# hvak/visual-underwater-slam

Measured on AMD Instinct MI355X. Metric: ORB detect+match frames/sec, higher is better.
Workload: dtype u8

## Files before the change

visual-underwater-slam_amd/csrc/orient.hip:

```cpp
#include "frontend_common.h"
#include <type_traits>
#define VUS_TABLE_QUAL __device__ constexpr
#include "../../include/vus_orb_tables.h"
#include "../../include/vus_tiled.h"

namespace {

#ifndef VUS_OR_WPE
#define VUS_OR_WPE 4
#endif
#ifndef VUS_OR_WPE_TILED
#define VUS_OR_WPE_TILED 7
#endif
constexpr int OR_R = 15;
constexpr int OR_ROWS = 2 * OR_R + 1;
constexpr int OR_DW = 10;
constexpr int BR_R = VUS_RBRIEF_REACH;
constexpr int BR_ROWS = 2 * BR_R + 1;
constexpr int BR_DW = 10;
constexpr int BR_DW_TILED = 16;
constexpr int OR_PC = 3;
constexpr int OR_NP = OR_ROWS * OR_PC;
constexpr int OR_KP_PER_WAVE = 8;

typedef uint32_t PatchVec __attribute__((ext_vector_type(2), aligned(1)));

template <int RADIUS, int DW, bool EXACT>
struct PatchRegs {
  static_assert(DW % 2 == 0, "row width must be a multiple of the vector width");
  static constexpr int ROWS = 2 * RADIUS + 1;
  static constexpr int HW = DW / 2;
  static constexpr int N = ROWS * HW;
  static constexpr int ITERS = (N + 63) / 64;
  PatchVec v[ITERS];
  uint32_t off[ITERS];

  __device__ __forceinline__ void init(int pitch, int lane) {
#pragma unroll
    for (int u = 0; u < ITERS; ++u) {
      const int t = min(lane + 64 * u, N - 1);
      off[u] = (uint32_t)((t / HW) * pitch + 8 * (t % HW));
    }
  }
  __device__ __forceinline__ void load(const uint8_t* __restrict__ src, int H, int W, int pitch, int y, int x,
                                       int lane) {
    const int xa = EXACT ? x - RADIUS : (x - RADIUS) & ~3;
    const bool inside = y - RADIUS >= 0 && y + RADIUS < H && xa >= 0 && xa + 4 * DW <= W;
    if (inside) {
      const uint8_t* base = src + (size_t)(y - RADIUS) * pitch + xa;
#pragma unroll
      for (int u = 0; u < ITERS; ++u) v[u] = *reinterpret_cast<const PatchVec*>(base + (size_t)off[u]);
    } else {
#pragma unroll
      for (int u = 0; u < ITERS; ++u) {
        const int t = min(lane + 64 * u, N - 1);
        const int r = t / HW, c = t - r * HW;
        const uint8_t* rp = src + (size_t)clampi(y - RADIUS + r, 0, H - 1) * pitch;
        const int gx = xa + 8 * c;
#pragma unroll
        for (int k = 0; k < 2; ++k)
          v[u][k] = (uint32_t)rp[clampi(gx + 4 * k, 0, W - 1)] | ((uint32_t)rp[clampi(gx + 4 * k + 1, 0, W - 1)] << 8) |
                    ((uint32_t)rp[clampi(gx + 4 * k + 2, 0, W - 1)] << 16) |
                    ((uint32_t)rp[clampi(gx + 4 * k + 3, 0, W - 1)] << 24);
      }
    }
  }
  __device__ __forceinline__ void store(uint32_t* __restrict__ dst, int lane) const {
#pragma unroll
    for (int u = 0; u < ITERS; ++u)
      if (lane + 64 * u < N) *reinterpret_cast<uint2*>(dst + 2 * (lane + 64 * u)) = make_uint2(v[u][0], v[u][1]);
  }
};

__device__ __forceinline__ uint4 tiled_piece_clamped(const uint8_t* __restrict__ src, int H, int W, int gy, int gx) {
  gy = clampi(gy, 0, H - 1);
  uint32_t w[4];
#pragma unroll
  for (int j = 0; j < 4; ++j) {
    w[j] = 0;
#pragma unroll
    for (int b = 0; b < 4; ++b) w[j] |= (uint32_t)src[vus_tiled_offset(gy, clampi(gx + 4 * j + b, 0, W - 1), W)] << (8 * b);
  }
  return make_uint4(w[0], w[1], w[2], w[3]);
}

struct PieceRC {
  int r, c;
};
constexpr int BR_PC = 3;
__host__ __device__ constexpr PieceRC disc_piece(int q) {
  const int c = (q >= OR_ROWS ? 1 : 0) + (q >= 2 * OR_ROWS ? 1 : 0);
  return {q - OR_ROWS * c, c};
}
constexpr int BR_SLOTS = 12 * ((BR_ROWS + 3) / 4);
__host__ __device__ constexpr PieceRC brief_piece(int t) {
  const int g = (t * 171) >> 11, w = t - 12 * g;
  return {4 * g + (w & 3), w >> 2};
}
template <int ROWS, int PC, int SLOTS, PieceRC (*PIECE)(int)>
constexpr bool dealing_is_a_permutation() {
  bool seen[ROWS * PC] = {};
  int n = 0;
  for (int s = 0; s < SLOTS; ++s) {
    const PieceRC p = PIECE(s);
    if (p.r < 0 || p.c < 0 || p.c >= PC) return false;
    if (p.r >= ROWS) continue;
    if (seen[p.r * PC + p.c]) return false;
    seen[p.r * PC + p.c] = true;
    ++n;
  }
  return n == ROWS * PC;
}
static_assert(dealing_is_a_permutation<OR_ROWS, OR_PC, OR_NP, disc_piece>(), "centroid patch: 31 x 3 pieces, one slot each");
static_assert(dealing_is_a_permutation<BR_ROWS, BR_PC, BR_SLOTS, brief_piece>(), "descriptor patch: 37 x 3 pieces, one slot each");
static_assert(BR_SLOTS <= 128, "descriptor patch: two wave-loads");

struct TiledDiscPair {
  static constexpr int ITERS = (2 * OR_NP + 63) / 64;
  static constexpr int SPLIT = OR_NP - 64;
  static_assert(ITERS == 3 && SPLIT > 0 && SPLIT < 64, "wave-load 1 is the only mixed one");
  static constexpr int PK_OFF_BITS = 10, PK_IDX_SHIFT = 10, PK_IDX_BITS = 10, PK_ROW_SHIFT = 20, PK_ROW_BITS = 6;
  static_assert(16 * (OR_ROWS - 1) + 128 * (OR_PC - 1) < (1 << PK_OFF_BITS) && PK_OFF_BITS <= PK_IDX_SHIFT, "pk: the offset field");
  static_assert(OR_NP - 1 < (1 << PK_IDX_BITS) && PK_IDX_SHIFT + PK_IDX_BITS <= PK_ROW_SHIFT, "pk: the weight index field");
  static_assert(OR_ROWS - 1 + 7 < (1 << PK_ROW_BITS) && PK_ROW_SHIFT + PK_ROW_BITS <= 32, "pk: the row field, nothing above it");
  uint4 v[ITERS];
  uint32_t pk[ITERS];

  static __device__ __forceinline__ int slot_of(int p) { return p >= OR_NP ? p - OR_NP : p; }
  __device__ __forceinline__ void init(int , int lane) {
#pragma unroll
    for (int u = 0; u < ITERS; ++u) {
      const PieceRC pc = disc_piece(slot_of(min(lane + 64 * u, 2 * OR_NP - 1)));
      const uint32_t r = (uint32_t)pc.r, c = (uint32_t)pc.c;
      pk[u] = r << PK_ROW_SHIFT | (OR_PC * r + c) << PK_IDX_SHIFT | (16u * r + 128u * c);
    }
  }
  __device__ __forceinline__ int row(int u) const { return (int)(pk[u] >> PK_ROW_SHIFT); }
  __device__ __forceinline__ int weight_index(int u) const { return (int)((pk[u] >> PK_IDX_SHIFT) & ((1u << PK_IDX_BITS) - 1u)); }
  static __device__ __forceinline__ bool inside(int H, int W, int y, int x) {
    const int xa = (x - OR_R) & ~15;
    return y - OR_R >= 0 && y + OR_R < H && xa >= 0 && xa + 16 * OR_PC <= W;
  }
  __device__ __forceinline__ void load(const uint8_t* __restrict__ src, int H, int W, int ya, int xa, int yb, int xb, bool b_live,
                                       int lane) {
    const bool second = lane >= SPLIT;
    const bool idle2 = lane >= 2 * OR_NP - 128;
    if (inside(H, W, ya, xa) && (!b_live || inside(H, W, yb, xb))) {
      const int y0a = ya - OR_R, y0b = yb - OR_R;
      const uint32_t koa = vus_tiled_offset(y0a & ~7, (xa - OR_R) & ~15, W) + 16u * (uint32_t)(y0a & 7);
      const uint32_t kob = b_live ? vus_tiled_offset(y0b & ~7, (xb - OR_R) & ~15, W) + 16u * (uint32_t)(y0b & 7) : koa;
      const uint32_t ysa = (uint32_t)(y0a & 7) << PK_ROW_SHIFT, ysb = (uint32_t)(y0b & 7) << PK_ROW_SHIFT, ystep = 8u * (uint32_t)W - 128u;
      constexpr int BLK = PK_ROW_SHIFT + 3;
      constexpr uint32_t OFF = (1u << PK_OFF_BITS) - 1u;
      v[0] = *reinterpret_cast<const uint4*>(src + koa + (size_t)(((pk[0] + ysa) >> BLK) * ystep + (pk[0] & OFF)));
      v[1] = make_uint4(0u, 0u, 0u, 0u);
      v[2] = make_uint4(0u, 0u, 0u, 0u);
      if (!second || b_live)
        v[1] = *reinterpret_cast<const uint4*>(
            src + (size_t)((second ? kob : koa) + ((pk[1] + (second ? ysb : ysa)) >> BLK) * ystep + (pk[1] & OFF)));
      if (b_live && !idle2)
        v[2] = *reinterpret_cast<const uint4*>(src + kob + (size_t)(((pk[2] + ysb) >> BLK) * ystep + (pk[2] & OFF)));
    } else {
#pragma unroll
      for (int u = 0; u < ITERS; ++u) {
        const int p = lane + 64 * u;
        const bool sec = p >= OR_NP;
        const PieceRC pc = disc_piece(slot_of(min(p, 2 * OR_NP - 1)));
        const int y = sec ? yb : ya, x = sec ? xb : xa;
        v[u] = make_uint4(0u, 0u, 0u, 0u);
        if (p < 2 * OR_NP && (!sec || b_live)) v[u] = tiled_piece_clamped(src, H, W, y - OR_R + pc.r, ((x - OR_R) & ~15) + 16 * pc.c);
      }
    }
  }
};

struct TiledBriefRegs {
  static constexpr int ROWS = BR_ROWS;
  uint4 v[2];
  uint32_t col;

  static __device__ __forceinline__ bool wide(int x) { return ((x - BR_R) & 15) > 11; }
  static __device__ __forceinline__ PieceRC loaded_piece(int lane, int u) {
    const PieceRC p = brief_piece(min(lane + 64 * u, BR_SLOTS - 1));
    return {min(p.r, ROWS - 1), p.c};
  }
  __device__ __forceinline__ void init(int , int ) { col = 0; }
  __device__ __forceinline__ void load(const uint8_t* __restrict__ src, int H, int W, int , int y, int x, int lane) {
    const int xa = (x - BR_R) & ~15, y0 = y - BR_R, rc = min(lane, ROWS - 1);
    const bool inside = y0 >= 0 && y + BR_R < H && xa >= 0 && xa + (wide(x) ? 64 : 48) <= W;
    if (inside) {
      const uint8_t* base = src + vus_tiled_offset(y0 & ~7, xa, W) + 16 * (y0 & 7);
      const uint32_t ys = (uint32_t)(y0 & 7), ystep = 8u * (uint32_t)W - 128u;
#pragma unroll
      for (int u = 0; u < 2; ++u) {
        const PieceRC p = loaded_piece(lane, u);
        const uint32_t off = (((uint32_t)p.r + ys) >> 3) * ystep + 16u * (uint32_t)p.r + 128u * (uint32_t)p.c;
        v[u] = *reinterpret_cast<const uint4*>(base + (size_t)off);
      }
      if (wide(x))
        col = *reinterpret_cast<const uint32_t*>(base + (size_t)((((uint32_t)rc + ys) >> 3) * ystep + 16u * (uint32_t)rc + 384u));
    } else {
#pragma unroll
      for (int u = 0; u < 2; ++u) {
        const PieceRC p = loaded_piece(lane, u);
        v[u] = tiled_piece_clamped(src, H, W, y0 + p.r, xa + 16 * p.c);
      }
      if (wide(x)) {
        const int gy = clampi(y0 + rc, 0, H - 1);
        uint32_t w = 0;
#pragma unroll
        for (int b = 0; b < 4; ++b) w |= (uint32_t)src[vus_tiled_offset(gy, clampi(xa + 48 + b, 0, W - 1), W)] << (8 * b);
        col = w;
      }
    }
  }
  __device__ __forceinline__ void store(uint32_t* __restrict__ dst, int lane, int x) const {
    uint4* d = reinterpret_cast<uint4*>(dst);
#pragma unroll
    for (int u = 0; u < 2; ++u) {
      const int t = lane + 64 * u;
      const PieceRC p = brief_piece(min(t, BR_SLOTS - 1));
      if (t < BR_SLOTS && p.r < ROWS) d[(BR_DW_TILED / 4) * p.r + p.c] = v[u];
    }
    if (wide(x) && lane < ROWS) dst[16 * lane + 12] = col;
  }
};

__device__ __forceinline__ int fold32(int x, int y) {
  auto r = __builtin_amdgcn_permlane32_swap((uint32_t)x, (uint32_t)y, false, false);
  return (int)(r[0] + r[1]);
}
__device__ __forceinline__ int fold16(int x, int y) {
  auto r = __builtin_amdgcn_permlane16_swap((uint32_t)x, (uint32_t)y, false, false);
  return (int)(r[0] + r[1]);
}
template <int CTRL>
__device__ __forceinline__ int dpp_i32(int v) { return __builtin_amdgcn_update_dpp(0, v, CTRL, 0xf, 0xf, true); }
constexpr int DPP_ROW_ROR8 = 0x128, DPP_HALF_MIRROR = 0x141, DPP_QUAD_XOR1 = 0xB1, DPP_QUAD_XOR2 = 0x4E;
__device__ __forceinline__ int fold8(int x, int y, bool upper8) {
  const int keep = upper8 ? y : x, give = upper8 ? x : y;
  return keep + dpp_i32<DPP_ROW_ROR8>(give);
}
__device__ __forceinline__ int allsum8(int v) {
  v += dpp_i32<DPP_HALF_MIRROR>(v);
  v += dpp_i32<DPP_QUAD_XOR1>(v);
  v += dpp_i32<DPP_QUAD_XOR2>(v);
  return v;
}
template <int CTRL>
__device__ __forceinline__ long long dpp_max_i64(long long key) {
  const int lo = dpp_i32<CTRL>((int)(uint32_t)key), hi = dpp_i32<CTRL>((int)(key >> 32));
  const long long ok = (long long)(((unsigned long long)(uint32_t)hi << 32) | (uint32_t)lo);
  return ok > key ? ok : key;
}
__device__ __forceinline__ long long allmax8_i64(long long key) {
  key = dpp_max_i64<DPP_HALF_MIRROR>(key);
  key = dpp_max_i64<DPP_QUAD_XOR1>(key);
  key = dpp_max_i64<DPP_QUAD_XOR2>(key);
  return key;
}

__device__ __forceinline__ uint32_t writelane_u32(uint32_t reg, uint32_t value, int lane_sel) {
  asm("s_mov_b32 m0, %2\n\tv_writelane_b32 %0, %1, m0" : "+v"(reg) : "s"(value), "s"(lane_sel));
  return reg;
}

__device__ __forceinline__ void load_bin_directions(const int (&cos_table)[VUS_N_ANGLE_BINS], const int (&sin_table)[VUS_N_ANGLE_BINS],
                                                    int lane, int (&bin_cos)[4], int (&bin_sin)[4]) {
#pragma unroll
  for (int q = 0; q < 4; ++q) {
    const int bq = min(4 * (lane & 7) + q, VUS_N_ANGLE_BINS - 1);
    bin_cos[q] = cos_table[bq];
    bin_sin[q] = sin_table[bq];
  }
}

struct RotOffTable {
  uint32_t v[VUS_N_ANGLE_BINS * 64 * 4];
};
constexpr RotOffTable make_rot_off_table(int row_bytes) {
  RotOffTable r{};
  for (int e = 0; e < VUS_N_ANGLE_BINS * 256; ++e) {
    const int bin = e / 256, test = e - 256 * bin, w = test >> 6, lane = test & 63;
    const int oa = VUS_RBRIEF_ROT[4 * e + 1] * row_bytes + VUS_RBRIEF_ROT[4 * e];
    const int ob = VUS_RBRIEF_ROT[4 * e + 3] * row_bytes + VUS_RBRIEF_ROT[4 * e + 2];
    r.v[(bin * 64 + lane) * 4 + w] = ((uint32_t)oa & 0xFFFFu) | ((uint32_t)ob << 16);
  }
  return r;
}
__device__ __attribute__((aligned(128))) const RotOffTable g_rot_off_table = make_rot_off_table(4 * BR_DW);
__device__ __attribute__((aligned(128))) const RotOffTable g_rot_off_table_tiled = make_rot_off_table(4 * BR_DW_TILED);

constexpr int OR_NV = OR_ROWS * (OR_DW / 2);
constexpr int OR_WT = 192;

template <int ALIGN>
struct DiscWeightTable {
  uint32_t v[ALIGN * OR_WT * 4];
};
struct DiscDwordWeight {
  uint32_t moment, count;
};
constexpr DiscDwordWeight disc_dword_weight(int dy, int dx0) {
  constexpr int umax[16] = {15, 15, 15, 15, 14, 14, 14, 13, 13, 12, 11, 10, 9, 8, 6, 3};
  DiscDwordWeight w{0u, 0u};
  if (dy < -OR_R || dy > OR_R) return w;
  const int um = umax[dy < 0 ? -dy : dy];
  for (int b = 0; b < 4; ++b) {
    const int dx = dx0 + b;
    if (dx >= -um && dx <= um) {
      w.moment |= (uint32_t)(dx + OR_R) << (8 * b);
      w.count |= 1u << (8 * b);
    }
  }
  return w;
}
template <int ALIGN>
constexpr DiscWeightTable<ALIGN> make_disc_weight_table() {
  DiscWeightTable<ALIGN> r{};
  for (int e = 0; e < ALIGN * OR_WT; ++e) {
    const int sh = e / OR_WT, t = e - sh * OR_WT;
    if (t >= OR_NV) continue;
    const int row = t / (OR_DW / 2), c = t - row * (OR_DW / 2);
    for (int d = 0; d < 2; ++d) {
      const DiscDwordWeight w = disc_dword_weight(row - OR_R, 4 * (2 * c + d) - sh - OR_R);
      r.v[4 * e + d] = w.moment;
      r.v[4 * e + 2 + d] = w.count;
    }
  }
  return r;
}
__device__ __attribute__((aligned(128))) const DiscWeightTable<4> g_disc_weight_table = make_disc_weight_table<4>();

constexpr int OR_WTD = 3 + 4 * (3 * 64 - OR_NP) + 4;
struct DiscWeightDwTable {
  uint32_t v[4 * OR_WTD * 2];
};
constexpr DiscWeightDwTable make_disc_weight_dw_table() {
  DiscWeightDwTable r{};
  for (int e = 0; e < 4 * OR_WTD; ++e) {
    const int a = e / OR_WTD, d = e - a * OR_WTD - 3;
    if (d < 0 || d >= OR_ROWS * 4 * OR_PC) continue;
    const int row = d / (4 * OR_PC), col = d - row * (4 * OR_PC);
    const DiscDwordWeight w = disc_dword_weight(row - OR_R, 4 * col - a - OR_R);
    r.v[2 * e] = w.moment;
    r.v[2 * e + 1] = w.count;
  }
  return r;
}
__device__ __attribute__((aligned(128))) const DiscWeightDwTable g_disc_weight_dw_table = make_disc_weight_dw_table();
constexpr bool disc_weight_dw_table_matches() {
  constexpr DiscWeightDwTable dw = make_disc_weight_dw_table();
  for (int sh = 0; sh < 16; ++sh)
    for (int q = 0; q < 3 * 64 - OR_NP; ++q)
      for (int d = 0; d < 4; ++d) {
        const int e = (sh & 3) * OR_WTD + 4 * q + d + 3 - (sh >> 2);
        const int r = q / OR_PC, c = q - r * OR_PC;
        const DiscDwordWeight w = disc_dword_weight(r - OR_R, 16 * c + 4 * d - sh - OR_R);
        if (dw.v[2 * e] != w.moment || dw.v[2 * e + 1] != w.count) return false;
      }
  return true;
}
static_assert(disc_weight_dw_table_matches(), "DiscWeightDwTable must weigh every dword as disc_dword_weight");

template <bool TILED, bool EXACT = false> struct OrGeom {
  static constexpr int ALIGN = 4, BR_DW = ::BR_DW;
  static constexpr int WT_VEC4 = ALIGN * OR_WT;
  static constexpr int GRP = 4, BLUR_BUF = 2;
  static constexpr bool BINS_AFTER_PHASE_A = false;
  typedef PatchRegs<OR_R, OR_DW, EXACT> Disc;
  typedef PatchRegs<BR_R, BR_DW, EXACT> Brief;
  static constexpr const uint32_t* WEIGHT_TABLE = g_disc_weight_table.v;
  static constexpr const uint32_t* ROT_TABLE = g_rot_off_table.v;
  static __device__ __forceinline__ uint4 disc_weights(const uint4* s_w, int sh, int lane, int u) {
    return s_w[sh * OR_WT + lane + 64 * u];
  }
};
template <bool EXACT> struct OrGeom<true, EXACT> {
  static_assert(!EXACT, "tiled planes are always read from aligned starts");
  static constexpr int ALIGN = 16, BR_DW = BR_DW_TILED;
  static constexpr int WT_VEC4 = 4 * OR_WTD * 2 / 4;
  static constexpr int GRP = 1, BLUR_BUF = 1;
  static constexpr bool BINS_AFTER_PHASE_A = true;
  typedef TiledDiscPair Disc;
  typedef TiledBriefRegs Brief;
  static constexpr const uint32_t* WEIGHT_TABLE = g_disc_weight_dw_table.v;
  static constexpr const uint32_t* ROT_TABLE = g_rot_off_table_tiled.v;
  static __device__ __forceinline__ void pair_moments(const uint4* s_w, const TiledDiscPair& pr, int sha, int shb, int lane, int& pa_a,
                                                      int& pq_a, int& pa_b, int& pq_b) {
    const bool second = lane >= TiledDiscPair::SPLIT;
    const int ea = (sha & 3) * OR_WTD + 3 - (sha >> 2), eb = (shb & 3) * OR_WTD + 3 - (shb >> 2);
    int mx[3], my[3];
#pragma unroll
    for (int u = 0; u < 3; ++u) {
      const int e = (u == 0 ? ea : u == 2 ? eb : second ? eb : ea) + 4 * pr.weight_index(u);
      const uint2* wd = reinterpret_cast<const uint2*>(s_w) + e;
      const uint32_t d[4] = {pr.v[u].x, pr.v[u].y, pr.v[u].z, pr.v[u].w};
      uint32_t sx = 0, rs = 0;
#pragma unroll
      for (int j = 0; j < 4; ++j) {
        const uint2 w = wd[j];
        sx = __builtin_amdgcn_udot4(d[j], w.x, sx, false);
        rs = __builtin_amdgcn_udot4(d[j], w.y, rs, false);
      }
      mx[u] = (int)sx - OR_R * (int)rs;
      my[u] = (pr.row(u) - OR_R) * (int)rs;
    }
    pa_a = mx[0] + (second ? 0 : mx[1]);
    pq_a = my[0] + (second ? 0 : my[1]);
    pa_b = mx[2] + (second ? mx[1] : 0);
    pq_b = my[2] + (second ? my[1] : 0);
  }
};
static_assert(2 * OR_R + 1 + 15 <= 16 * OR_PC && 2 * BR_R + 1 + 11 <= 48 && 2 * BR_R + 1 + 15 <= 52 && 52 <= 4 * BR_DW_TILED,
              "tiled patch rows: 16-byte aligned starts; descriptor rows of 48 bytes for a <= 11, 52 beyond");
static_assert(sizeof(DiscWeightDwTable) == 16 * OrGeom<true>::WT_VEC4, "LDS copy of the tiled weights: whole uint4");

constexpr int OO_CELL = 64, OO_MAX_CELLS = 1024;
__global__ __launch_bounds__(256) void orient_order_kernel(const uint32_t* __restrict__ kp_keys, const int* __restrict__ kp_count,
                                                           int max_kp, int W, int cw, int n_cells, int* __restrict__ order) {
  __shared__ int s_cnt[OO_MAX_CELLS];
  __shared__ int s_wave[4];
  const int n = blockIdx.x, tid = threadIdx.x;
  const int cnt = clampi(kp_count[n], 0, max_kp);
  const uint32_t* keys = kp_keys + (size_t)n * max_kp;
  int* ord = order + (size_t)n * max_kp;
  for (int r = tid; r < n_cells; r += 256) s_cnt[r] = 0;
  __syncthreads();
  for (int j = tid; j < cnt; j += 256) {
    const uint32_t pos = keys[j] & VUS_KEY_POS_MASK;
    const int y = (int)(pos / (uint32_t)W), x = (int)(pos - (uint32_t)y * (uint32_t)W);
    atomicAdd(&s_cnt[(y / OO_CELL) * cw + (x / OO_CELL)], 1);
  }
  __syncthreads();
  int c[4], sum = 0;
#pragma unroll
  for (int q = 0; q < 4; ++q) {
    c[q] = 4 * tid + q < n_cells ? s_cnt[4 * tid + q] : 0;
    sum += c[q];
  }
  int incl = sum;
#pragma unroll
  for (int d = 1; d < 64; d <<= 1) {
    const int o = __shfl_up(incl, d);
    if ((tid & 63) >= d) incl += o;
  }
  if ((tid & 63) == 63) s_wave[tid >> 6] = incl;
  __syncthreads();
  int base = incl - sum;
  for (int w = 0; w < (tid >> 6); ++w) base += s_wave[w];
#pragma unroll
  for (int q = 0; q < 4; ++q)
    if (4 * tid + q < n_cells) {
      s_cnt[4 * tid + q] = base;
      base += c[q];
    }
  __syncthreads();
  for (int j = tid; j < cnt; j += 256) {
    const uint32_t pos = keys[j] & VUS_KEY_POS_MASK;
    const int y = (int)(pos / (uint32_t)W), x = (int)(pos - (uint32_t)y * (uint32_t)W);
    ord[atomicAdd(&s_cnt[(y / OO_CELL) * cw + (x / OO_CELL)], 1)] = j;
  }
  for (int j = cnt + tid; j < max_kp; j += 256) ord[j] = j;
}

}

extern "C" int vus_orient_order(const uint32_t* kp_keys, const int* kp_count, int n_img, int max_kp, int H, int W, int* order,
                                void* stream) {
  VUS_REQUIRE(kp_keys && kp_count && order, "null buffer");
  VUS_REQUIRE(n_img >= 0 && max_kp >= 1 && H >= 1 && W >= 1, "n_img=%d max_kp=%d H=%d W=%d", n_img, max_kp, H, W);
  if (n_img == 0) return VUS_OK;
  int cw = (W + OO_CELL - 1) / OO_CELL, ch = (H + OO_CELL - 1) / OO_CELL;
  VUS_REQUIRE((long long)cw * ch <= OO_MAX_CELLS, "image of %d x %d pixels has more than %d cells of %d x %d", W, H, OO_MAX_CELLS,
              OO_CELL, OO_CELL);
  orient_order_kernel<<<n_img, 256, 0, vus::as_stream(stream)>>>(kp_keys, kp_count, max_kp, W, cw, cw * ch, order);
  VUS_CHECK_LAUNCH("orient_order");
  return VUS_OK;
}

namespace {

template <bool EXACT, bool ORDERED, bool TILED>
__global__ __launch_bounds__(256) __attribute__((amdgpu_waves_per_eu(TILED ? VUS_OR_WPE_TILED : VUS_OR_WPE, 8))) void orient_rbrief_kernel(
    const uint8_t* __restrict__ img, const uint8_t* __restrict__ blur, int H, int W, int pitch,
    const uint32_t* __restrict__ kp_keys, const int* __restrict__ kp_count, int max_kp, const int* __restrict__ order,
    uint64_t* __restrict__ desc_out, uint8_t* __restrict__ angle_out, int n_img, int chunks_per_img) {
  typedef OrGeom<TILED, EXACT> G;
  __shared__ uint4 s_w[G::WT_VEC4];
  __shared__ __attribute__((aligned(TILED ? 16 : 8))) uint32_t s_blur[4][G::BLUR_BUF][BR_ROWS * G::BR_DW];
  const int lane = threadIdx.x & 63;
  const int wave = __builtin_amdgcn_readfirstlane(threadIdx.x >> 6);
  const int xcd = blockIdx.x & 7, slot = blockIdx.x >> 3;
  const int n = (slot / chunks_per_img) * 8 + xcd;
  const int chunk = slot - (slot / chunks_per_img) * chunks_per_img;
  if (n >= n_img) return;
  {
    const uint4* wt = reinterpret_cast<const uint4*>(G::WEIGHT_TABLE);
#pragma unroll
    for (int i = 0; i < (G::WT_VEC4 + 255) / 256; ++i)
      if (G::WT_VEC4 % 256 == 0 || threadIdx.x + 256 * i < G::WT_VEC4) s_w[threadIdx.x + 256 * i] = wt[threadIdx.x + 256 * i];
  }
  const uint8_t* im = img + (size_t)n * H * pitch;
  const uint8_t* bl = blur + (size_t)n * H * W;
  const int base_i = (chunk * 4 + wave) * OR_KP_PER_WAVE;
  const int n_live = clampi(min(kp_count[n], max_kp) - base_i, 0, OR_KP_PER_WAVE);
  int my_y = 0, my_x = 0;
  int my_idx = base_i + lane;
  if (ORDERED && lane < OR_KP_PER_WAVE && base_i + lane < max_kp) my_idx = order[(size_t)n * max_kp + base_i + lane];
  if (lane < n_live) {
    const uint32_t pos = kp_keys[(size_t)n * max_kp + my_idx] & VUS_KEY_POS_MASK;
    my_y = (int)(pos / (uint32_t)W);
    my_x = (int)(pos - (uint32_t)my_y * (uint32_t)W);
  }
  int bin_cos[4], bin_sin[4];
  if constexpr (!G::BINS_AFTER_PHASE_A) load_bin_directions(VUS_ANGLE_COS, VUS_ANGLE_SIN, lane, bin_cos, bin_sin);
  constexpr int GRP = G::GRP;
  typename G::Disc pr[GRP];
  typename G::Brief pb;
#pragma unroll
  for (int kk = 0; kk < GRP; ++kk) pr[kk].init(pitch, lane);
  pb.init(W, lane);
  int mom_dy[3];
  if constexpr (!TILED) {
#pragma unroll
    for (int u = 0; u < 3; ++u) mom_dy[u] = min(lane + 64 * u, OR_NV - 1) / (OR_DW / 2) - OR_R;
  }
  __syncthreads();
  if (n_live == 0) {
    if (lane < 4 * OR_KP_PER_WAVE && base_i + (lane >> 2) < max_kp) desc_out[((size_t)n * max_kp + base_i) * 4 + lane] = 0;
    if (lane < OR_KP_PER_WAVE && base_i + lane < max_kp) angle_out[(size_t)n * max_kp + base_i + lane] = 0;
    return;
  }

  int pa[8], pq[8];
  if constexpr (TILED) {
#pragma unroll
    for (int g = 0; g < 4; ++g) {
      const int ya = __builtin_amdgcn_readlane(my_y, 2 * g), xa = __builtin_amdgcn_readlane(my_x, 2 * g);
      const int yb = __builtin_amdgcn_readlane(my_y, 2 * g + 1), xb = __builtin_amdgcn_readlane(my_x, 2 * g + 1);
      pa[2 * g] = pq[2 * g] = pa[2 * g + 1] = pq[2 * g + 1] = 0;
      if (2 * g < n_live) pr[0].load(im, H, W, ya, xa, yb, xb, 2 * g + 1 < n_live, lane);
      if (2 * g < n_live)
        G::pair_moments(s_w, pr[0], (xa - OR_R) & 15, (xb - OR_R) & 15, lane, pa[2 * g], pq[2 * g], pa[2 * g + 1], pq[2 * g + 1]);
    }
    pb.load(bl, H, W, W, __builtin_amdgcn_readlane(my_y, 0), __builtin_amdgcn_readlane(my_x, 0), lane);
  } else {
#pragma unroll
    for (int g = 0; g < 8 / GRP; ++g) {
#pragma unroll
      for (int kk = 0; kk < GRP; ++kk) {
        const int k = GRP * g + kk;
        if (k < n_live) pr[kk].load(im, H, W, pitch, __builtin_amdgcn_readlane(my_y, k), __builtin_amdgcn_readlane(my_x, k), lane);
      }
      if (g == 8 / GRP - 1)
        pb.load(bl, H, W, W, __builtin_amdgcn_readlane(my_y, 0), __builtin_amdgcn_readlane(my_x, 0), lane);
#pragma unroll
      for (int kk = 0; kk < GRP; ++kk) {
        const int k = GRP * g + kk;
        pa[k] = 0;
        pq[k] = 0;
        if (k < n_live) {
          const int sh = EXACT ? 0 : (__builtin_amdgcn_readlane(my_x, k) - OR_R) & (G::ALIGN - 1);
          uint32_t sx = 0;
          int si = 0, sy = 0;
#pragma unroll
          for (int u = 0; u < 3; ++u) {
            const uint4 w = G::disc_weights(s_w, sh, lane, u);
            sx = __builtin_amdgcn_udot4(pr[kk].v[u][0], w.x, sx, false);
            sx = __builtin_amdgcn_udot4(pr[kk].v[u][1], w.y, sx, false);
            uint32_t rs = __builtin_amdgcn_udot4(pr[kk].v[u][0], w.z, 0u, false);
            rs = __builtin_amdgcn_udot4(pr[kk].v[u][1], w.w, rs, false);
            si += (int)rs;
            sy += mom_dy[u] * (int)rs;
          }
          pa[k] = (int)sx - OR_R * si;
          pq[k] = sy;
        }
      }
    }
  }
  if constexpr (G::BINS_AFTER_PHASE_A) load_bin_directions(VUS_ANGLE_COS, VUS_ANGLE_SIN, lane, bin_cos, bin_sin);
  int m10, m01;
  {
    const bool up8 = (lane & 8) != 0;
    int c[4], d[2];
#pragma unroll
    for (int j = 0; j < 4; ++j) c[j] = fold32(pa[j], pa[j + 4]);
#pragma unroll
    for (int j = 0; j < 2; ++j) d[j] = fold16(c[j], c[j + 2]);
    m10 = allsum8(fold8(d[0], d[1], up8));
#pragma unroll
    for (int j = 0; j < 4; ++j) c[j] = fold32(pq[j], pq[j + 4]);
#pragma unroll
    for (int j = 0; j < 2; ++j) d[j] = fold16(c[j], c[j + 2]);
    m01 = allsum8(fold8(d[0], d[1], up8));
  }
  int my_bin;
  {
    long long best = (long long)(-0x7FFFFFFFFFFFFFFFll - 1);
#pragma unroll
    for (int q = 0; q < 4; ++q) {
      const int bq = 4 * (lane & 7) + q;
      long long key = ((long long)m10 * bin_cos[q] + (long long)m01 * bin_sin[q]) * 32 + (31 - bq);
      if (bq >= VUS_N_ANGLE_BINS) key = (long long)(-0x7FFFFFFFFFFFFFFFll - 1);
      best = key > best ? key : best;
    }
    best = allmax8_i64(best);
    my_bin = 31 - (int)(best & 31);
  }
  {
    const int j_ang = ORDERED ? __shfl(my_idx, lane >> 3) : base_i + (lane >> 3);
    if ((lane & 7) == 0 && base_i + (lane >> 3) < max_kp) angle_out[(size_t)n * max_kp + j_ang] = (uint8_t)my_bin;
  }

  uint32_t wlo = 0, whi = 0;
  const uint4* rot = reinterpret_cast<const uint4*>(G::ROT_TABLE) + lane;
  uint4 to = rot[__builtin_amdgcn_readlane(my_bin, 0) * 64];
  for (int k = 0; k < n_live; ++k) {
    uint32_t* patch = s_blur[wave][k & (G::BLUR_BUF - 1)];
    if constexpr (TILED) pb.store(patch, lane, __builtin_amdgcn_readlane(my_x, k));
    else pb.store(patch, lane);
    const uint4 cto = to;
    const int cx = __builtin_amdgcn_readlane(my_x, k);
    if (k + 1 < n_live) {
      pb.load(bl, H, W, W, __builtin_amdgcn_readlane(my_y, k + 1), __builtin_amdgcn_readlane(my_x, k + 1), lane);
      to = rot[__builtin_amdgcn_readlane(my_bin, 8 * (k + 1)) * 64];
    }
    __builtin_amdgcn_fence(__ATOMIC_ACQ_REL, "wavefront");
    const int sh_blur = EXACT ? 0 : (cx - BR_R) & (G::ALIGN - 1);
    const uint8_t* c = reinterpret_cast<const uint8_t*>(patch) + BR_R * (4 * G::BR_DW) + BR_R + sh_blur;
    const uint32_t tw[4] = {cto.x, cto.y, cto.z, cto.w};
#pragma unroll
    for (int w = 0; w < 4; ++w) {
      const int a = c[(int16_t)(tw[w] & 0xFFFFu)];
      const int b = c[(int16_t)(tw[w] >> 16)];
      const uint64_t word = __ballot(a < b);
      wlo = writelane_u32(wlo, (uint32_t)word, 4 * k + w);
      whi = writelane_u32(whi, (uint32_t)(word >> 32), 4 * k + w);
    }
    __builtin_amdgcn_fence(__ATOMIC_ACQ_REL, "wavefront");
  }
  const int j_desc = ORDERED ? __shfl(my_idx, lane >> 2) : 0;
  if (lane < 4 * OR_KP_PER_WAVE && base_i + (lane >> 2) < max_kp)
    desc_out[ORDERED ? ((size_t)n * max_kp + j_desc) * 4 + (lane & 3) : ((size_t)n * max_kp + base_i) * 4 + lane] =
        ((uint64_t)whi << 32) | wlo;
}

}

static int orient_launch(bool tiled, const uint8_t* img, const uint8_t* blur, int n_img, int H, int W, int pitch,
                         const uint32_t* kp_keys, const int* kp_count, int max_kp, const int* order, uint64_t* desc_out,
                         uint8_t* angle_out, void* stream) {
  if (int rc = check_image_args(img, n_img, H, W, pitch)) return rc;
  if (tiled)
    if (int rc = check_tiled_args(img, blur, H, W)) return rc;
  VUS_REQUIRE(blur && kp_keys && kp_count && desc_out && angle_out, "null buffer");
  VUS_REQUIRE(max_kp >= 1, "max_kp=%d", max_kp);
  if (n_img == 0) return VUS_OK;
  const int chunks = (max_kp + 4 * OR_KP_PER_WAVE - 1) / (4 * OR_KP_PER_WAVE);
  const long long blocks = (long long)((n_img + 7) / 8) * 8 * chunks;
  VUS_REQUIRE(blocks < (1ll << 31), "too many workgroups (%lld)", blocks);
  const bool aligned = ((reinterpret_cast<uintptr_t>(img) | reinterpret_cast<uintptr_t>(blur) | (uintptr_t)pitch |
                         (uintptr_t)W | ((uintptr_t)H * (uintptr_t)pitch)) & 3u) == 0;
  auto launch = [&](auto exact, auto ordered, auto tiled_planes) {
    orient_rbrief_kernel<decltype(exact)::value, decltype(ordered)::value, decltype(tiled_planes)::value>
        <<<(unsigned)blocks, 256, 0, vus::as_stream(stream)>>>(img, blur, H, W, pitch, kp_keys, kp_count, max_kp, order, desc_out,
                                                               angle_out, n_img, chunks);
  };
  constexpr std::true_type yes{};
  constexpr std::false_type no{};
  if (!tiled && aligned) order ? launch(no, yes, no) : launch(no, no, no);
  else if (!tiled) order ? launch(yes, yes, no) : launch(yes, no, no);
  else order ? launch(no, yes, yes) : launch(no, no, yes);
  VUS_CHECK_LAUNCH(tiled ? "orient_rbrief_tiled" : "orient_rbrief");
  return VUS_OK;
}

extern "C" int vus_orient_rbrief(const uint8_t* img, const uint8_t* blur, int n_img, int H, int W, int pitch,
                                 const uint32_t* kp_keys, const int* kp_count, int max_kp,
                                 uint64_t* desc_out, uint8_t* angle_out, void* stream) {
  return orient_launch(false, img, blur, n_img, H, W, pitch, kp_keys, kp_count, max_kp, nullptr, desc_out, angle_out, stream);
}

extern "C" int vus_orient_rbrief_ordered(const uint8_t* img, const uint8_t* blur, int n_img, int H, int W, int pitch,
                                         const uint32_t* kp_keys, const int* kp_count, int max_kp, const int* order,
                                         uint64_t* desc_out, uint8_t* angle_out, void* stream) {
  VUS_REQUIRE(order != nullptr, "null buffer");
  return orient_launch(false, img, blur, n_img, H, W, pitch, kp_keys, kp_count, max_kp, order, desc_out, angle_out, stream);
}

extern "C" int vus_orient_rbrief_tiled(const uint8_t* img_tiled, const uint8_t* blur_tiled, int n_img, int H, int W,
                                       const uint32_t* kp_keys, const int* kp_count, int max_kp, const int* order,
                                       uint64_t* desc_out, uint8_t* angle_out, void* stream) {
  return orient_launch(true, img_tiled, blur_tiled, n_img, H, W, W, kp_keys, kp_count, max_kp, order, desc_out, angle_out, stream);
}
```

Before: 216,700.

## Fold disc weight table by row symmetry, pad descriptor LDS rows, pin waves per EU

```diff
diff --git a/visual-underwater-slam_amd/csrc/orient.hip b/visual-underwater-slam_amd/csrc/orient.hip
--- a/visual-underwater-slam_amd/csrc/orient.hip
+++ b/visual-underwater-slam_amd/csrc/orient.hip
@@ -11,6 +11,9 @@
 #endif
 #ifndef VUS_OR_WPE_TILED
 #define VUS_OR_WPE_TILED 7
+#endif
+#ifndef VUS_OR_WPE_TILED_MAX
+#define VUS_OR_WPE_TILED_MAX 7
 #endif
 constexpr int OR_R = 15;
 constexpr int OR_ROWS = 2 * OR_R + 1;
@@ -18,10 +21,12 @@
 constexpr int BR_R = VUS_RBRIEF_REACH;
 constexpr int BR_ROWS = 2 * BR_R + 1;
 constexpr int BR_DW = 10;
-constexpr int BR_DW_TILED = 16;
+constexpr int BR_DW_TILED = 20;
 constexpr int OR_PC = 3;
 constexpr int OR_NP = OR_ROWS * OR_PC;
 constexpr int OR_KP_PER_WAVE = 8;
+constexpr int OR_WFOLD = OR_R + 1;
+constexpr int OR_WROW = 4 * OR_PC + 1;
 
 typedef uint32_t PatchVec __attribute__((ext_vector_type(2), aligned(1)));
 
@@ -92,7 +97,10 @@
   const int c = (q >= OR_ROWS ? 1 : 0) + (q >= 2 * OR_ROWS ? 1 : 0);
   return {q - OR_ROWS * c, c};
 }
-constexpr int BR_SLOTS = 12 * ((BR_ROWS + 3) / 4);
+__host__ __device__ constexpr int disc_weight_entry(int r, int c) { return OR_WROW * (r < OR_ROWS - 1 - r ? r : OR_ROWS - 1 - r) + 4 * c; }
+constexpr int BR_GROUP_ROWS = 4;
+constexpr int BR_SLOTS = BR_GROUP_ROWS * BR_PC * ((BR_ROWS + BR_GROUP_ROWS - 1) / BR_GROUP_ROWS);
+static_assert(BR_GROUP_ROWS == 4 && BR_GROUP_ROWS * BR_PC == 12, "brief_piece divides by 12 and by 4 with shifts");
 __host__ __device__ constexpr PieceRC brief_piece(int t) {
   const int g = (t * 171) >> 11, w = t - 12 * g;
   return {4 * g + (w & 3), w >> 2};
@@ -121,7 +129,7 @@
   static_assert(ITERS == 3 && SPLIT > 0 && SPLIT < 64, "wave-load 1 is the only mixed one");
   static constexpr int PK_OFF_BITS = 10, PK_IDX_SHIFT = 10, PK_IDX_BITS = 10, PK_ROW_SHIFT = 20, PK_ROW_BITS = 6;
   static_assert(16 * (OR_ROWS - 1) + 128 * (OR_PC - 1) < (1 << PK_OFF_BITS) && PK_OFF_BITS <= PK_IDX_SHIFT, "pk: the offset field");
-  static_assert(OR_NP - 1 < (1 << PK_IDX_BITS) && PK_IDX_SHIFT + PK_IDX_BITS <= PK_ROW_SHIFT, "pk: the weight index field");
+  static_assert(disc_weight_entry(OR_R, OR_PC - 1) < (1 << PK_IDX_BITS) && PK_IDX_SHIFT + PK_IDX_BITS <= PK_ROW_SHIFT, "pk: the weight entry field");
   static_assert(OR_ROWS - 1 + 7 < (1 << PK_ROW_BITS) && PK_ROW_SHIFT + PK_ROW_BITS <= 32, "pk: the row field, nothing above it");
   uint4 v[ITERS];
   uint32_t pk[ITERS];
@@ -132,11 +140,11 @@
     for (int u = 0; u < ITERS; ++u) {
       const PieceRC pc = disc_piece(slot_of(min(lane + 64 * u, 2 * OR_NP - 1)));
       const uint32_t r = (uint32_t)pc.r, c = (uint32_t)pc.c;
-      pk[u] = r << PK_ROW_SHIFT | (OR_PC * r + c) << PK_IDX_SHIFT | (16u * r + 128u * c);
+      pk[u] = r << PK_ROW_SHIFT | (uint32_t)disc_weight_entry(pc.r, pc.c) << PK_IDX_SHIFT | (16u * r + 128u * c);
     }
   }
   __device__ __forceinline__ int row(int u) const { return (int)(pk[u] >> PK_ROW_SHIFT); }
-  __device__ __forceinline__ int weight_index(int u) const { return (int)((pk[u] >> PK_IDX_SHIFT) & ((1u << PK_IDX_BITS) - 1u)); }
+  __device__ __forceinline__ int weight_entry(int u) const { return (int)((pk[u] >> PK_IDX_SHIFT) & ((1u << PK_IDX_BITS) - 1u)); }
   static __device__ __forceinline__ bool inside(int H, int W, int y, int x) {
     const int xa = (x - OR_R) & ~15;
     return y - OR_R >= 0 && y + OR_R < H && xa >= 0 && xa + 16 * OR_PC <= W;
@@ -222,7 +230,7 @@
       const PieceRC p = brief_piece(min(t, BR_SLOTS - 1));
       if (t < BR_SLOTS && p.r < ROWS) d[(BR_DW_TILED / 4) * p.r + p.c] = v[u];
     }
-    if (wide(x) && lane < ROWS) dst[16 * lane + 12] = col;
+    if (wide(x) && lane < ROWS) dst[BR_DW_TILED * lane + 12] = col;
   }
 };
 
@@ -332,7 +340,7 @@
 }
 __device__ __attribute__((aligned(128))) const DiscWeightTable<4> g_disc_weight_table = make_disc_weight_table<4>();
 
-constexpr int OR_WTD = 3 + 4 * (3 * 64 - OR_NP) + 4;
+constexpr int OR_WTD = 3 + OR_WROW * OR_WFOLD + 4;
 struct DiscWeightDwTable {
   uint32_t v[4 * OR_WTD * 2];
 };
@@ -340,8 +348,9 @@
   DiscWeightDwTable r{};
   for (int e = 0; e < 4 * OR_WTD; ++e) {
     const int a = e / OR_WTD, d = e - a * OR_WTD - 3;
-    if (d < 0 || d >= OR_ROWS * 4 * OR_PC) continue;
-    const int row = d / (4 * OR_PC), col = d - row * (4 * OR_PC);
+    if (d < 0 || d >= OR_WROW * OR_WFOLD) continue;
+    const int row = d / OR_WROW, col = d - row * OR_WROW;
+    if (col >= 4 * OR_PC) continue;
     const DiscDwordWeight w = disc_dword_weight(row - OR_R, 4 * col - a - OR_R);
     r.v[2 * e] = w.moment;
     r.v[2 * e + 1] = w.count;
@@ -352,13 +361,14 @@
 constexpr bool disc_weight_dw_table_matches() {
   constexpr DiscWeightDwTable dw = make_disc_weight_dw_table();
   for (int sh = 0; sh < 16; ++sh)
-    for (int q = 0; q < 3 * 64 - OR_NP; ++q)
-      for (int d = 0; d < 4; ++d) {
-        const int e = (sh & 3) * OR_WTD + 4 * q + d + 3 - (sh >> 2);
-        const int r = q / OR_PC, c = q - r * OR_PC;
-        const DiscDwordWeight w = disc_dword_weight(r - OR_R, 16 * c + 4 * d - sh - OR_R);
-        if (dw.v[2 * e] != w.moment || dw.v[2 * e + 1] != w.count) return false;
-      }
+    for (int r = 0; r < OR_ROWS; ++r)
+      for (int c = 0; c < OR_PC; ++c)
+        for (int d = 0; d < 4; ++d) {
+          const int e = (sh & 3) * OR_WTD + disc_weight_entry(r, c) + d + 3 - (sh >> 2);
+          if (e < 0 || e >= 4 * OR_WTD) return false;
+          const DiscDwordWeight w = disc_dword_weight(r - OR_R, 16 * c + 4 * d - sh - OR_R);
+          if (dw.v[2 * e] != w.moment || dw.v[2 * e + 1] != w.count) return false;
+        }
   return true;
 }
 static_assert(disc_weight_dw_table_matches(), "DiscWeightDwTable must weigh every dword as disc_dword_weight");
@@ -393,7 +403,7 @@
     int mx[3], my[3];
 #pragma unroll
     for (int u = 0; u < 3; ++u) {
-      const int e = (u == 0 ? ea : u == 2 ? eb : second ? eb : ea) + 4 * pr.weight_index(u);
+      const int e = (u == 0 ? ea : u == 2 ? eb : second ? eb : ea) + pr.weight_entry(u);
       const uint2* wd = reinterpret_cast<const uint2*>(s_w) + e;
       const uint32_t d[4] = {pr.v[u].x, pr.v[u].y, pr.v[u].z, pr.v[u].w};
       uint32_t sx = 0, rs = 0;
@@ -414,6 +424,8 @@
 };
 static_assert(2 * OR_R + 1 + 15 <= 16 * OR_PC && 2 * BR_R + 1 + 11 <= 48 && 2 * BR_R + 1 + 15 <= 52 && 52 <= 4 * BR_DW_TILED,
               "tiled patch rows: 16-byte aligned starts; descriptor rows of 48 bytes for a <= 11, 52 beyond");
+static_assert(BR_DW_TILED % 4 == 0 && (BR_ROWS - 1) * 4 * BR_DW_TILED + 52 < (1 << 15),
+              "descriptor patch in LDS: rows of whole uint4, every byte offset an int16 of g_rot_off_table_tiled");
 static_assert(sizeof(DiscWeightDwTable) == 16 * OrGeom<true>::WT_VEC4, "LDS copy of the tiled weights: whole uint4");
 
 constexpr int OO_CELL = 64, OO_MAX_CELLS = 1024;
@@ -482,7 +494,7 @@
 namespace {
 
 template <bool EXACT, bool ORDERED, bool TILED>
-__global__ __launch_bounds__(256) __attribute__((amdgpu_waves_per_eu(TILED ? VUS_OR_WPE_TILED : VUS_OR_WPE, 8))) void orient_rbrief_kernel(
+__global__ __launch_bounds__(256) __attribute__((amdgpu_waves_per_eu(TILED ? VUS_OR_WPE_TILED : VUS_OR_WPE, TILED ? VUS_OR_WPE_TILED_MAX : 8))) void orient_rbrief_kernel(
     const uint8_t* __restrict__ img, const uint8_t* __restrict__ blur, int H, int W, int pitch,
     const uint32_t* __restrict__ kp_keys, const int* __restrict__ kp_count, int max_kp, const int* __restrict__ order,
     uint64_t* __restrict__ desc_out, uint8_t* __restrict__ angle_out, int n_img, int chunks_per_img) {
```

After: 222,500, median of 6. +2.7%, better.
